# zju3dv/PVO

Hardware: AMD Instinct MI355X
Metric: VO keyframe updates/sec (8-keyframe window, 512x384, 36 edges; 6 graph updates + edge rebuild per keyframe) (higher is better)
Workload: dtype f16 (volume, lookup, update operator) / f32 (BA assembly) / f64 (pose solve); 1 GPU; S-B: BASELINE.json configs[1] window (8 keyframes, 48x64 maps, E=36, itrs=2), synthetic; edges=36, parallelism=independent window per GPU

## Files before the change

### include/pvo_hip.h

```cpp
#ifndef PVO_HIP_H
#define PVO_HIP_H

#include <stddef.h>
#include <stdint.h>

#ifdef __cplusplus
extern "C" {
#endif

enum { PVO_F32 = 0, PVO_F16 = 1, PVO_BF16 = 2, PVO_F64 = 3 };

enum {
  PVO_OK = 0,
  PVO_EINVAL = 1,
  PVO_ELAUNCH = 2,
  PVO_EWORKSPACE = 3,
  PVO_EUNSUPPORTED = 4
};

const char* pvo_strerror(int code);
const char* pvo_last_hip_error(void);
#define PVO_ABI_VERSION 106
int pvo_version(void);
size_t pvo_graph_update_args_size(void);
// ... 536 lines not shown
                 int t0, int t1, int iterations, float lm, float ep, int motion_only,
                 float* dx_out, float* dz_out, int dz_rows, int* status_out,
                 void* workspace, size_t workspace_bytes,
                 const float* disps_sens, float alpha, void* stream);
int pvo_ba_stereo(void* workspace, size_t workspace_bytes, int E, int P, int nframes, int HW, float baseline, void* stream);
int pvo_ba_rig(float* poses, float* disps, const float* intrinsics,
               const float* targets, const float* weights, const float* eta,
               const int64_t* ii, const int64_t* jj,
               int E, int nframes, int ht, int wd, int K_eta,
               int t0, int t1, int iterations, float lm, float ep, int motion_only,
               float* dx_out, float* dz_out, int dz_rows, int* status_out,
               void* workspace, size_t workspace_bytes,
               const float* disps_sens, float alpha, float baseline, void* stream);
int pvo_ba_last_partition(void* workspace, size_t workspace_bytes, int E, int P, int nframes, int HW, int* out, void* stream);
int pvo_ba_local(const float* poses, const float* disps, const float* intrinsics,
                 const float* targets, const float* weights, const float* eta,
                 const int64_t* ii, const int64_t* jj,
                 int E, int nframes, int ht, int wd, int K_eta, int t0, int t1,
                 int motion_only, void* sys,
                 void* workspace, size_t workspace_bytes, void* stream);
int pvo_ba_finish(float* poses, float* disps, void* sys,
                  const int64_t* ii, const int64_t* jj,
                  int E, int nframes, int ht, int wd, int t0, int t1,
                  float lm, float ep, int motion_only, int clamp_frames, float disp_min,
                  float* dx_out, float* dz_out, int dz_rows, int* status_out,
                  void* workspace, size_t workspace_bytes, void* stream);
int pvo_ba_finish_graph(float* poses, float* disps, void* sys,
                        const int64_t* ii, const int64_t* jj,
                        int E, int nframes, int ht, int wd, int t0, int t1,
                        float lm, float ep, int motion_only, int clamp_frames, float disp_min,
                        float* dx_out, float* dz_out, int dz_rows, int* status_out,
                        void* workspace, size_t workspace_bytes, int graph_edges, void* stream);
int pvo_ba_solve_kind(int P, int graph_edges, int packed);
int pvo_ba_sigma(const void* sys, void* workspace, size_t workspace_bytes,
                 const int64_t* ii, const int64_t* jj,
                 int E, int P, int nframes, int ht, int wd, int t0, float lm, float ep,
                 double* pose_cov, float* var_cond, float* var_pose, int* status_out, void* stream);
int pvo_ba_uncertainty(const float* poses, const float* disps, const float* intrinsics,
                       const float* targets, const float* weights, const float* eta,
                       const int64_t* ii, const int64_t* jj,
                       int E, int nframes, int ht, int wd, int K_eta,
                       int t0, int t1, float lm, float ep,
                       double* pose_cov, float* var_cond, float* var_pose, int* status_out,
                       void* workspace, size_t workspace_bytes,
                       const float* disps_sens, float alpha, float baseline, void* stream);
size_t pvo_ba_calib_workspace_bytes(int E, int P, int nframes, int HW);
int pvo_ba_calib(float* poses, float* disps, float* intrinsics,
                 const float* targets, const float* weights, const float* eta,
                 const int64_t* ii, const int64_t* jj,
                 int E, int nframes, int ht, int wd, int K_eta,
                 int t0, int t1, int iterations, float lm, float ep, float ep_c, int free_mask,
                 float* dx_out, float* dz_out, int dz_rows, float* dc_out, int* status_out,
                 void* workspace, size_t workspace_bytes, void* calib_workspace, size_t calib_bytes, void* stream);
size_t pvo_ba_packed_elems(const int* first_host, int P);
int pvo_ba_pack(void* sys, const int* first_s, void* msg, int P, void* stream);
int pvo_ba_finish_packed(float* poses, float* disps, const void* msg, const int* first_s,
                         const int64_t* ii, const int64_t* jj,
                         int E, int nframes, int ht, int wd, int t0, int t1,
                         float lm, float ep, int motion_only, int clamp_frames, float disp_min,
                         float* dx_out, float* dz_out, int dz_rows, int* status_out,
                         void* workspace, size_t workspace_bytes, void* stream);

typedef struct pvo_ba_riders {
  const void* cx; const void* cw; const float* cbias; void* cy; long long crows; int cCout; int cdtype;
  const void* gnet; const void* gw; const float* gbias; float* gpart; int gE; int gHW; int gdtype;
  const float* xpart; const float* xwt; const float* xbias; float* xg; int xE; int xchunks;
// ... 35 lines not shown
```

### pvo_amd/_lib.py

```python
import ctypes
import os

_HERE = os.path.dirname(os.path.abspath(__file__))
LIB_PATH = os.path.join(_HERE, "libpvo_hip.so")

PVO_F32, PVO_F16, PVO_BF16, PVO_F64 = 0, 1, 2, 3
PVO_ABI_VERSION = 106

_c = ctypes
_vp, _i, _f, _sz = _c.c_void_p, _c.c_int, _c.c_float, _c.c_size_t

SIGNATURES = {
    "pvo_strerror": (_c.c_char_p, [_i]),
    "pvo_version": (_i, []),
    "pvo_graph_update_args_size": (_sz, []),
    "pvo_last_hip_error": (_c.c_char_p, []),
    "pvo_debug_config": (_i, [_i, _i]),
    "pvo_knob": (_i, [_i]),
    "pvo_debug_trunk_range": (_i, [_i, _vp, _vp, _vp, _vp, _vp, _i, _i, _i, _i, _i, _i, _i, _i, _i, _vp, _i, _i, _vp]),
    "pvo_corr_index_forward": (_i, [_vp, _vp, _vp, _i, _i, _i, _i, _i, _i, _i, _vp]),
    "pvo_corr_index_backward": (_i, [_vp, _vp, _vp, _i, _i, _i, _i, _i, _i, _i, _vp]),
    "pvo_corr_pyramid_lookup": (_i, [_vp, _vp, _vp, _i, _i, _i, _i, _i, _i, _i, _i, _i, _vp, _i, _vp]),
    "pvo_altcorr_forward": (_i, [_vp, _vp, _vp, _vp, _i, _i, _i, _i, _i, _i, _i, _i, _i, _vp]),
    "pvo_altcorr_backward": (_i, [_vp, _vp, _vp, _vp, _vp, _vp, _i, _i, _i, _i, _i, _i, _i, _i, _i, _vp]),
# ... 96 lines not shown
    "pvo_tsdf_sparse_mesh_args_size": (_sz, []),
    "pvo_tsdf_sparse_mesh_workspace_bytes": (_sz, [_i]),
    "pvo_tsdf_sparse_mesh": (_i, [_vp, _vp, _sz, _vp]),
    "pvo_tsdf_panoptic_args_size": (_sz, []),
    "pvo_tsdf_mesh_labels_args_size": (_sz, []),
    "pvo_tsdf_integrate_panoptic": (_i, [_vp, _vp, _vp, _sz, _vp]),
    "pvo_tsdf_sparse_integrate_panoptic": (_i, [_vp, _vp, _vp, _sz, _vp]),
    "pvo_tsdf_mesh_panoptic": (_i, [_vp, _vp, _vp, _sz, _vp]),
    "pvo_tsdf_sparse_mesh_panoptic": (_i, [_vp, _vp, _vp, _sz, _vp]),
    "pvo_tsdf_render_args_size": (_sz, []),
    "pvo_tsdf_render_workspace_bytes": (_sz, [_i]),
    "pvo_tsdf_render": (_i, [_vp, _vp, _sz, _vp]),
    "pvo_tsdf_sparse_render_args_size": (_sz, []),
    "pvo_tsdf_sparse_render_workspace_bytes": (_sz, [_i]),
    "pvo_tsdf_sparse_render": (_i, [_vp, _vp, _sz, _vp]),
    "pvo_tsdf_track_args_size": (_sz, []),
    "pvo_tsdf_track_workspace_bytes": (_sz, [_i, _i, _i]),
    "pvo_tsdf_track": (_i, [_vp, _vp, _sz, _vp]),
    "pvo_tsdf_sparse_track_args_size": (_sz, []),
    "pvo_tsdf_sparse_track_workspace_bytes": (_sz, [_i, _i, _i]),
    "pvo_tsdf_sparse_track": (_i, [_vp, _vp, _sz, _vp]),
    "pvo_ba_last_partition": (_i, [_vp, _sz, _i, _i, _i, _i, ctypes.POINTER(ctypes.c_int), _vp]),
    "pvo_ba_packed_elems": (_sz, [ctypes.POINTER(ctypes.c_int), _i]),
    "pvo_ba_pack": (_i, [_vp, _vp, _vp, _i, _vp]),
    "pvo_ba_finish_packed": (_i, [_vp, _vp, _vp, _vp, _vp, _vp, _i, _i, _i, _i, _i, _i, _f, _f, _i, _i, _f,
                                  _vp, _vp, _i, _vp, _vp, _sz, _vp]),
    "pvo_ba_local": (_i, [_vp, _vp, _vp, _vp, _vp, _vp, _vp, _vp, _i, _i, _i, _i, _i, _i, _i,
                          _i, _vp, _vp, _sz, _vp]),
    "pvo_ba_finish": (_i, [_vp, _vp, _vp, _vp, _vp, _i, _i, _i, _i, _i, _i, _f, _f, _i, _i, _f,
                           _vp, _vp, _i, _vp, _vp, _sz, _vp]),
    "pvo_ba_finish_graph": (_i, [_vp, _vp, _vp, _vp, _vp, _i, _i, _i, _i, _i, _i, _f, _f, _i, _i, _f,
                                 _vp, _vp, _i, _vp, _vp, _sz, _i, _vp]),
    "pvo_ba_solve_kind": (_i, [_i, _i, _i]),
    "pvo_ba_finish_riders": (_i, [_vp, _vp, _vp, _vp, _vp, _i, _i, _i, _i, _i, _i, _f, _f, _i, _i, _f,
                                  _vp, _vp, _i, _vp, _vp, _sz, _vp, _vp]),
    "pvo_ba_finish_conv1x1": (_i, [_vp, _vp, _vp, _vp, _vp, _i, _i, _i, _i, _i, _i, _f, _f, _i, _i, _f,
                                   _vp, _vp, _i, _vp, _vp, _sz, _vp, _vp, _vp, _vp, _c.c_longlong, _i, _i, _vp]),
    "pvo_ba_train_workspace_bytes": (_sz, [_i, _i, _i, _i, _i, _i]),
    "pvo_ba_train_vjp_scratch_bytes": (_sz, [_i, _i, _i, _i, _i, _i]),
    "pvo_ba_train": (_i, [_vp, _vp, _vp, _vp, _vp, _vp, _vp, _vp, _vp, _vp, _vp, _vp, _i, _i, _i, _i, _i, _i, _i,
                          _vp, _vp, _vp, _vp, _sz, _i, _vp]),
    "pvo_ba_train_vjp": (_i, [_vp, _vp, _vp, _vp, _vp, _vp, _vp, _vp, _vp, _vp, _vp, _i, _i, _i, _i, _i, _i, _i,
                              _vp, _vp, _vp, _vp, _vp, _vp, _vp, _vp, _sz, _vp, _sz, _i, _vp]),
}



class UpdateWeights(_c.Structure):
    _fields_ = [("dtype", _i), ("flags", _i)] + [(n, _vp) for n in (
        "enc0_w", "enc0_b", "cenc2_w", "cenc2_b", "fenc0_w", "fenc0_b", "fenc2_w", "fenc2_b", "glo_w", "glo_b",
        "gate_wt", "gate_b", "zr_w", "q_w", "zr_inp_w", "q_inp_w", "heads1_w", "heads1_b", "heads2_w", "heads2_b",
        "agg1_w", "agg1_b", "agg2_w", "agg2_b", "eta_w", "eta_b", "up_w", "up_b")]


class OperatorArgs(_c.Structure):
    _fields_ = [("E", _i), ("H", _i), ("W", _i), ("levels", _vp * 4), ("slots", _vp), ("num_slots", _i),
                ("coords", _vp), ("corr", _vp), ("motion", _vp), ("net", _vp), ("net_out", _vp), ("inp", _vp),
                ("P_zr", _vp), ("P_q", _vp), ("static_by_slot", _i), ("seg_ptr", _vp), ("seg_idx", _vp), ("K", _i), ("heads", _vp),
                ("eta_frame", _vp), ("eta_pos", _vp), ("R", _i), ("damping", _vp), ("EP", _f), ("eta_scale", _f), ("eta", _vp),
                ("upmask", _vp)]


class GraphUpdateArgs(_c.Structure):
    _fields_ = [("op", OperatorArgs), ("nframes", _i), ("poses", _vp), ("disps", _vp), ("intrinsics", _vp),
                ("ii", _vp), ("jj", _vp), ("target", _vp), ("delta_dy", _vp), ("raw_mask", _vp), ("weight", _vp),
                ("full_flow", _vp), ("segm", _vp), ("max_segments", _i), ("vote_thresh", _f), ("dy_thresh", _f),
# ... 170 lines not shown
```

### pvo_amd/csrc/ba.hip

```cpp
#include "se3.h"
#include "conv1x1_tile.h"
#include "glo_tile.h"
#include <stdlib.h>
#include <type_traits>
#include "ba_workspace.h"
#include "ba_assemble.h"
#include "ba_schur.h"

namespace {

#ifdef PVO_BA_PROBE
__device__ unsigned long long* g_ba_probe = nullptr;
#define BA_PROBE(slot) do { if (g_ba_probe && threadIdx.x == 0) g_ba_probe[slot] = __builtin_readcyclecounter(); } while (0)
#else
#define BA_PROBE(slot)
#endif
#if defined(PVO_BA_PROBE) && PVO_BA_PROBE == 2
#define BA_PROBE_STEP(slot) do { if (g_ba_probe && lane == 0 && kb == P / 2) g_ba_probe[slot] = __builtin_readcyclecounter(); } while (0)
#else
#define BA_PROBE_STEP(slot)
#endif

__device__ __forceinline__ double rsqrt_nr(double d) {
  double y = __builtin_amdgcn_rsq(d);
// ... 1603 lines not shown
  __syncthreads();
  if (tid < 64) {
    for (int j = nc - 1; j >= 0; --j) {
      if (lane == j) xk[j] = s[j] * rinv[j];
      const double xj = xk[j];
      if (lane < j) s[lane] -= Lk[j][lane] * xj;
    }
  }
  __syncthreads();
  const int bj = blockIdx.x;
  if (bj == kb) {
    if (tid < nc) xvec[c0 + tid] = xk[tid];
    return;
  }
  if (tid < kNB) {
    const int col = kNB * bj + tid;
    double v = yrow[col];
    for (int r = 0; r < nc; ++r) v -= A[static_cast<size_t>(c0 + r) * n + col] * xk[r];
    yrow[col] = v;
  }
}

__global__ __launch_bounds__(256) void dense_finish_kernel(const double* __restrict__ xvec, float* __restrict__ poses, float* __restrict__ dx_ws,
                                                           float* __restrict__ dx_out, int* __restrict__ meta, int* __restrict__ status_out,
                                                           int P, int t0, Riders riders) {
  extern __shared__ __attribute__((aligned(16))) unsigned char smem[];
  if (blockIdx.x > 0) {
    ride(smem, riders, blockIdx.x - 1);
    return;
  }
  solve_epilogue([&](int i) { return xvec[i]; }, meta[4] | meta[2], true, 0, P, t0, poses, dx_ws, dx_out, meta, status_out, true, [] {});
}

template <bool CALIB>
__device__ __forceinline__ void ba_backsub_body(
    const Plan& pl, const int64_t* __restrict__ jj, const float* __restrict__ Ei, const float* __restrict__ Eij,
    const float* __restrict__ Q, const float* __restrict__ w, const float* __restrict__ dx,
    float* __restrict__ disps, float* __restrict__ dz_out, int dz_rows, int HW, int t0, int P,
    int clamp_frames, float disp_min, const float* __restrict__ Gc = nullptr, const float* __restrict__ dcw = nullptr) {
  const int k = blockIdx.y;
  const int x = blockIdx.x * 256 + threadIdx.x;
  __shared__ int s_edge[256], s_pose[256];
  __shared__ float s_dx[256][6];
  const bool live = k < pl.meta[0] && !pl.meta[2];
  const int e0 = live ? pl.eptr[k] : 0, deg = live ? pl.eptr[k + 1] - e0 : 0;
  const bool in_lds = deg <= 255;
  constexpr int lo = 1;
  if (live && in_lds && static_cast<int>(threadIdx.x) <= deg) {
    const int r = static_cast<int>(threadIdx.x) - 1;
    int e = 0, p;
    if (r < 0) p = pl.kx[k] - t0;
    else { e = pl.eidx[e0 + r]; p = static_cast<int>(jj[e]) - t0; }
    const bool ok = p >= 0 && p < P && p >= lo;
    s_edge[threadIdx.x] = e; s_pose[threadIdx.x] = ok ? p : -1;
#pragma unroll
    for (int n = 0; n < 6; ++n) s_dx[threadIdx.x][n] = ok ? dx[6 * p + n] : 0.0f;
  }
  BA_WG_PROBE(2, 0);
  __syncthreads();
  BA_WG_PROBE(2, 1);
  if (x >= HW) return;
  if (k < clamp_frames && pl.kidx[k] < 0) {
    const float v = disps[static_cast<long long>(k) * HW + x];
    if (v < disp_min) disps[static_cast<long long>(k) * HW + x] = disp_min;
  }
  if constexpr (CALIB) {
    if (k >= pl.meta[0]) return;
    if (!live || reinterpret_cast<const int*>(dcw)[4] != 0) {
      if (dz_out && k < dz_rows) dz_out[static_cast<long long>(k) * HW + x] = 0.0f;
      return;
    }
  }
  if (!live) return;
  float acc = 0.0f;
  if (in_lds) {
    for (int q = 0; q <= deg; ++q) {
      const int p = s_pose[q];
      if (p < 0) continue;
      const float* base = (q == 0) ? Ei + static_cast<long long>(p) * 6 * HW : Eij + static_cast<long long>(s_edge[q]) * 6 * HW;
      float sacc = 0.0f;
#pragma unroll
      for (int n = 0; n < 6; ++n) sacc += base[static_cast<long long>(n) * HW + x] * s_dx[q][n];
      acc += sacc;
    }
  } else {
    for (int r = -1; r < deg; ++r) {
      const RowRef R = row_of(r, k, pl, Ei, Eij, jj, HW, t0, P);
      if (R.pose < lo) continue;
      float sacc = 0.0f;
#pragma unroll
      for (int n = 0; n < 6; ++n) sacc += R.base[static_cast<long long>(n) * HW + x] * dx[6 * R.pose + n];
      acc += sacc;
    }
  }
  if constexpr (CALIB) {
    float cacc = 0.0f;
#pragma unroll
    for (int n = 0; n < 4; ++n) cacc += Gc[(static_cast<long long>(k) * 4 + n) * HW + x] * dcw[n];
    acc += cacc;
  }
  const float dz = Q[static_cast<long long>(k) * HW + x] * (w[static_cast<long long>(k) * HW + x] - acc);
  float d = disps[static_cast<long long>(pl.kx[k]) * HW + x] + dz;
  if (pl.kx[k] < clamp_frames && d < disp_min) d = disp_min;
  disps[static_cast<long long>(pl.kx[k]) * HW + x] = d;
  if (dz_out && k < dz_rows) dz_out[static_cast<long long>(k) * HW + x] = dz;
  BA_WG_PROBE(2, 2);
}

__global__ __launch_bounds__(256) void ba_backsub_kernel(
    Plan pl, const int64_t* __restrict__ jj, const float* __restrict__ Ei, const float* __restrict__ Eij,
    const float* __restrict__ Q, const float* __restrict__ w, const float* __restrict__ dx,
    float* __restrict__ disps, float* __restrict__ dz_out, int dz_rows, int HW, int t0, int P,
    int clamp_frames, float disp_min) {
  ba_backsub_body<false>(pl, jj, Ei, Eij, Q, w, dx, disps, dz_out, dz_rows, HW, t0, P, clamp_frames, disp_min);
}

constexpr int kSigmaMaxPoses = 64;
constexpr int kSigmaBlocks = 210;

__global__ __launch_bounds__(256) void ba_sigma_prepare_kernel(const long long* __restrict__ sys, double* __restrict__ out, int n, float lm, float ep) {
  const int idx = blockIdx.x * 256 + threadIdx.x;
  if (idx >= n * n) return;
  const int r = idx / n, c = idx - r * n;
  if (r > c) { out[idx] = 0.0; return; }
  double v = static_cast<double>(sys[static_cast<long long>(c) * n + r]) * kInvFix;
  if (r == c) v += static_cast<double>(ep) + static_cast<double>(lm) * v;
  out[idx] = v;
}

__global__ __launch_bounds__(1024) void ba_sigma_factor_kernel(double* R, int n, const int* __restrict__ meta, int* __restrict__ status_out) {
  __shared__ double s_col[8][8];
  int* flag = reinterpret_cast<int*>(R + static_cast<long long>(n) * n);
  double* rdiag = R + static_cast<long long>(n) * n + 1;
  const int tid = threadIdx.x, c = tid >> 7, il = tid & 127;
  int failed = (meta[2] | meta[3] | meta[4]) ? 1 : 0;
  for (int j0 = 0; j0 < n && !failed; j0 += 8) {
    const int j = j0 + c;
    double acc[3] = {0.0, 0.0, 0.0};
    for (int k0 = 0; k0 < j0; k0 += 8) {
      __syncthreads();
      if (tid < 64) s_col[tid >> 3][tid & 7] = (j0 + (tid & 7) < n) ? R[static_cast<long long>(k0 + (tid >> 3)) * n + j0 + (tid & 7)] : 0.0;
      __syncthreads();
#pragma unroll
      for (int kk = 0; kk < 8; ++kk) {
        const double a = s_col[kk][c];
        const double* row = R + static_cast<long long>(k0 + kk) * n;
#pragma unroll
        for (int u = 0; u < 3; ++u) {
// ... 675 lines not shown
    const bool stage2 = dense_window;
#define PVO_SCHUR_LAUNCH(V, PX) hipLaunchKernelGGL((ba_schur_mfma_kernel<V, PX>), sgrid, dim3(256), (PX == 256 ? sdyn : 0), st, w.plan, jj, eta, K_eta, w.Eii, w.Cii, w.bz, w.Ei, \
                                                   w.Eij, w.Q, w.w, sys, HW, t0, P, two_stage ? w.part : nullptr, ii, E, chunksA, deal_rows, w.Mrg, depth_done, (PX == 256 ? lds_floats : 0), \
                                                   (stage2 && PX == 256) ? w.spart : nullptr, w.srow, stage2 ? w.sT : nullptr, disps)
    if ((HW & 3) == 0) { if (pix == 256) PVO_SCHUR_LAUNCH(true, 256); else if (pix == 512) PVO_SCHUR_LAUNCH(true, 512); else PVO_SCHUR_LAUNCH(true, 1024); }
    else { if (pix == 256) PVO_SCHUR_LAUNCH(false, 256); else if (pix == 512) PVO_SCHUR_LAUNCH(false, 512); else PVO_SCHUR_LAUNCH(false, 1024); }
#undef PVO_SCHUR_LAUNCH
    PVO_CHECK_LAUNCH();
    if (stage2) {
      hipLaunchKernelGGL(ba_schur_reduce_kernel, dim3(kSchurStagePairs, Kgrid), dim3(256), 0, st, w.plan, w.spart, w.srow, w.sT, sys, gx, 6 * P, t0);
      PVO_CHECK_LAUNCH();
    }
  }
  return PVO_OK;
}

enum SolveKind { kSolveStatus, kSolveDense, kSolveEnvelope, kSolveChain, kSolveBlocks };
struct SolveForm { SolveKind kind; int chol; };
static SolveForm solve_form(int P, int E, bool packed, int knob) {
  if (P == 0) return {kSolveStatus, 0};
  if (knob >= 1 && knob <= 3) return {kSolveChain, knob - 1};
  if (knob == 4) return {kSolveEnvelope, 2};
  if (knob == 6 && !packed) return {kSolveBlocks, 0};
  if (P <= kDenseMaxPoses) return {kSolveDense, 0};
  if (knob != 5 && !packed && static_cast<long long>(E) > 8LL * P) return {kSolveBlocks, 0};
  return {kSolveEnvelope, 2};
}

extern "C" int pvo_ba_solve_kind(int P, int graph_edges, int packed) {
  if (P < 0 || graph_edges < 0) return -1;
  return static_cast<int>(solve_form(P, graph_edges, packed != 0, pvo_knob(PVO_KNOB_BA_SOLVER)).kind);
}

static int ba_finish_impl(float* poses, float* disps, void* sys_, const long long* msg, const int* first_s,
                          const int64_t* ii, const int64_t* jj,
                          int E, int nframes, int ht, int wd, int t0, int t1,
                          float lm, float ep, int motion_only, int clamp_frames, float disp_min,
                          float* dx_out, float* dz_out, int dz_rows, int* status_out,
                          void* workspace, size_t workspace_bytes,
                          const pvo_ba_riders* jobs, int graph_edges, void* stream) {
  Riders rider{};
  size_t rider_lds = 0;
  if (jobs && jobs->cy && jobs->crows > 0) {
    if (!jobs->cx || !jobs->cw || jobs->cCout <= 0 || jobs->cCout % 192) return PVO_EINVAL;
    if (jobs->cdtype != PVO_F16 && jobs->cdtype != PVO_BF16) return PVO_EUNSUPPORTED;
    if (pvo_misaligned16(jobs->cx, jobs->cw, jobs->cy)) return PVO_EINVAL;
    if (jobs->crows > (1LL << 24)) return PVO_EUNSUPPORTED;
    rider.cx = static_cast<const uint16_t*>(jobs->cx); rider.cw = static_cast<const uint16_t*>(jobs->cw); rider.cbias = jobs->cbias;
    rider.cy = static_cast<uint16_t*>(jobs->cy); rider.crows = jobs->crows; rider.cCout = jobs->cCout; rider.cdtype = jobs->cdtype;
    rider.crow_blocks = static_cast<int>((jobs->crows + 63) / 64);
    rider.cblocks = rider.crow_blocks * (jobs->cCout / 192);
    rider_lds = c1t::kTileBytes;
  }
  if (jobs && jobs->gpart && jobs->gE > 0 && jobs->gHW > 0) {
    if (!jobs->gnet || !jobs->gw || jobs->gE > 65535) return PVO_EINVAL;
    if (jobs->gdtype != PVO_F16 && jobs->gdtype != PVO_BF16) return PVO_EUNSUPPORTED;
    if (pvo_misaligned16(jobs->gnet, jobs->gw)) return PVO_EINVAL;
    rider.gnet = static_cast<const uint16_t*>(jobs->gnet); rider.gw = static_cast<const uint16_t*>(jobs->gw); rider.gbias = jobs->gbias;
    rider.gpart = jobs->gpart; rider.gHW = jobs->gHW; rider.gchunks = (jobs->gHW + 255) / 256; rider.gdtype = jobs->gdtype;
    rider.gblocks = jobs->gE * rider.gchunks;
    if (rider_lds < static_cast<size_t>(glt::kTileBytes)) rider_lds = glt::kTileBytes;
  }
  if (jobs && jobs->xg && jobs->xE > 0) {
    if (!jobs->xpart || !jobs->xwt || !jobs->xbias || jobs->xchunks <= 0) return PVO_EINVAL;
    rider.xpart = jobs->xpart; rider.xwt = jobs->xwt; rider.xbias = jobs->xbias; rider.xg = jobs->xg;
    rider.xchunks = jobs->xchunks; rider.xblocks = jobs->xE;
    if (rider_lds < 512) rider_lds = 512;
  }
  const int rider_blocks = rider.cblocks + rider.gblocks + rider.xblocks;
  int rc = check_common(E, nframes, ht, wd, t0, t1);
  if (rc != PVO_OK) return rc;
  if (clamp_frames < 0 || clamp_frames > nframes) return PVO_EINVAL;
  const int P = t1 - t0, HW = ht * wd;
  long long* sys = static_cast<long long*>(sys_);
  if (!poses || !disps || (!sys && !msg) || !workspace) return PVO_EINVAL;
  if (P > kMaxEnvBlocks) return PVO_EUNSUPPORTED;
  Ws w;
  if (!carve_checked(&w, workspace, workspace_bytes, E, P, nframes, HW)) return PVO_EWORKSPACE;
  hipStream_t st = pvo_stream(stream);
  const int n6 = 6 * P;
  const SolveForm form = solve_form(P, graph_edges >= 0 ? graph_edges : E, msg != nullptr, pvo_knob(PVO_KNOB_BA_SOLVER));
  if (msg && form.kind == kSolveStatus) return PVO_OK;
  constexpr size_t kSolveLdsMax = 142000;
  if (form.kind == kSolveDense) {
    const size_t dl = dense_lds_bytes(n6);
    const size_t lds = dl > rider_lds ? dl : rider_lds;
    const int Td = dense_N(n6) / 16;
    if (!pvo_allow_lds<ba_solve_dense_kernel<4>>(kSolveLdsMax) || !pvo_allow_lds<ba_solve_dense_kernel<14>>(kSolveLdsMax) ||
        !pvo_allow_lds<ba_solve_dense_kernel<17>>(kSolveLdsMax))
      return PVO_ELAUNCH;
    const auto kernel = Td <= 5 ? ba_solve_dense_kernel<4> : (Td <= 10 ? ba_solve_dense_kernel<14> : ba_solve_dense_kernel<17>);
    hipLaunchKernelGGL(kernel, dim3(1 + rider_blocks), dim3(256), lds, st, sys, msg, first_s, poses, w.dx, dx_out, w.plan.meta, status_out,
                       P, t0, lm, ep, rider);
  } else if (form.kind == kSolveEnvelope || form.kind == kSolveChain) {
    int* part = form.kind == kSolveEnvelope ? reinterpret_cast<int*>(w.xchg) : nullptr;
    if (msg) {
      hipLaunchKernelGGL(ba_env_packed_kernel, dim3(P), dim3(256), 0, st, msg, first_s, w.plan.env, n6);
      hipLaunchKernelGGL(ba_prepare_packed_kernel, dim3(P + 1), dim3(256), 0, st, msg, first_s, w.chol, w.plan.env, n6, lm, ep,
                         static_cast<long long>(kSolveLdsMax), part);
    } else {
      hipLaunchKernelGGL(ba_env_kernel, dim3((n6 * n6 + 2047) / 2048), dim3(256), 0, st, sys, w.plan.env, n6);
      hipLaunchKernelGGL(ba_prepare_kernel, dim3((n6 * n6 + n6 + 2047) / 2048), dim3(256), 0, st, sys, w.chol, w.plan.env, n6, lm, ep,
                         static_cast<long long>(kSolveLdsMax), part);
    }
    PVO_CHECK_LAUNCH();
    if (!part && hipMemsetAsync(w.xchg, 0, 16, st) != hipSuccess) return PVO_ELAUNCH;
    if (!pvo_allow_lds<ba_solve_twin_kernel>(kSolveLdsMax)) return PVO_ELAUNCH;
    hipLaunchKernelGGL(ba_solve_twin_kernel, dim3(2 + rider_blocks), dim3(256), kSolveLdsMax > rider_lds ? kSolveLdsMax : rider_lds, st,
                       w.chol, poses, w.dx, dx_out, w.plan.meta, status_out, P, t0, w.plan.env, static_cast<long long>(kSolveLdsMax), w.xchg,
                       form.chol, rider);
  } else {
    if (form.kind == kSolveBlocks) {
      hipLaunchKernelGGL(ba_prepare_kernel, dim3((n6 * n6 + n6 + 2047) / 2048), dim3(256), 0, st, sys, w.chol, w.plan.env, n6, lm, ep,
                         0LL , static_cast<int*>(nullptr));
      PVO_CHECK_LAUNCH();
      if (hipMemsetAsync(w.xchg, 0, 16, st) != hipSuccess) return PVO_ELAUNCH;
// ... 281 lines not shown
```

### pvo_amd/csrc/ba_workspace.h

```cpp
#pragma once
#include "common.h"

namespace {

constexpr float kMinDepth = 0.25f;

constexpr double kFix = 268435456.0, kInvFix = 1.0 / 268435456.0;
__device__ __forceinline__ void fix_add(long long* sys, long long idx, double v, int* meta) {
  if (!(fabs(v) < 3.0e10)) { meta[4] = 1; return; }
#ifdef PVO_BA_NO_ATOMICS
  if (idx >= 0) return;
#endif
  atomicAdd(reinterpret_cast<unsigned long long*>(sys + idx), static_cast<unsigned long long>(__double2ll_rn(v * kFix)));
}
constexpr int kDealEdges = 2;
constexpr int kPPT = 2;
constexpr int kChunkA = 256 * kPPT;
constexpr int kMaxSep = 12;
constexpr int kXchgDoubles = 2 + 36 * kMaxSep * kMaxSep + 12 * kMaxSep;


#if defined(PVO_BA_PROBE) && PVO_BA_PROBE == 3
__device__ unsigned long long* g_ba_wg_probe = nullptr;
#define BA_WG_PROBE(kern, slot)                                                                                         \
  do {                                                                                                                  \
    if (g_ba_wg_probe && threadIdx.x == 0 && blockIdx.z == 0) {                                                         \
      const unsigned wg_ = blockIdx.y * gridDim.x + blockIdx.x;                                                         \
      if (wg_ < 4096u) g_ba_wg_probe[((kern) * 4096u + wg_) * 8u + (slot)] = wall_clock64();                            \
    }                                                                                                                   \
  } while (0)
#else
#define BA_WG_PROBE(kern, slot)
#endif

struct Plan {
  int* kidx;
  int* kx;
  int* eptr;
  int* eidx;
  int* meta;
  int* env;
};

struct Ws {
  Plan plan;
  float *Eii, *Eij;
  float *Cii, *bz;
  float *Ei;
  float *Q, *w;
  float *dx;
  float *part;
  long long* sys;
  double* chol;
  double* xchg;
  double* ldiag;
  double* xvec;
  float* Mrg;
  float* spart;
  short* srow;
  int* sT;
  size_t bytes;
};
constexpr int kSchurStagePairs = 36;
constexpr int kSchurStageFront = 8;
__host__ __device__ __forceinline__ int schur_stage_frames(int P) { return (P > 0 && P <= 29) ? P + kSchurStageFront : 0; }
__host__ __device__ __forceinline__ int schur_stage_slot(int frame, int t0, int P) {
  const int slot = frame - t0 + kSchurStageFront;
  return (slot >= 0 && slot < schur_stage_frames(P)) ? slot : -1;
}

__host__ size_t align_up(size_t x) { return (x + 255) & ~static_cast<size_t>(255); }

__host__ Ws carve(void* base, int E, int P, int F, int HW) {
  Ws w{};
  char* p = static_cast<char*>(base);
// ... 69 lines not shown
  int cnt = 0;
  for (int f = lo; f < hi; ++f) cnt += pl.kidx[f];
  seg[tid + 1] = cnt;
  if (tid == 0) seg[0] = 0;
  __syncthreads();
  if (tid == 0) for (int i = 1; i <= 256; ++i) seg[i] += seg[i - 1];
  __syncthreads();
  int run = seg[tid];
  for (int f = lo; f < hi; ++f) {
    if (pl.kidx[f]) { pl.kx[run] = f; pl.kidx[f] = run; ++run; } else pl.kidx[f] = -1;
  }
  const int K = seg[256];
  __syncthreads();
  for (int k = tid; k < K; k += 256) {
    const int f = pl.kx[k];
    int c = 0;
    for (int e = 0; e < E; ++e) c += (ii[e] == f) ? 1 : 0;
    pl.eptr[k + 1] = c;
  }
  if (tid == 0) pl.eptr[0] = 0;
  __syncthreads();
  if (tid == 0) for (int k = 1; k <= K; ++k) pl.eptr[k] += pl.eptr[k - 1];
  __syncthreads();
  for (int k = tid; k < K; k += 256) {
    const int f = pl.kx[k];
    int o = pl.eptr[k];
    for (int e = 0; e < E; ++e) if (ii[e] == f) pl.eidx[o++] = e;
  }
  if (tid == 0) {
    pl.meta[0] = K;
    pl.meta[1] = 0;
    pl.meta[3] = 0;
    pl.meta[4] = 0;
    pl.meta[2] = (!motion_only && K_eta != K && K_eta != 1) ? 1 : 0;
    store_prior(pl.meta, sens, alpha);
    pl.meta[8] = __float_as_int(baseline);
  }
}

}
```

### pvo_amd/droid_backends.py

```python
import ctypes
import itertools

import torch

from . import _lib
from ._lib import PvoHipError, check

_DT = {torch.float32: _lib.PVO_F32, torch.float16: _lib.PVO_F16,
       torch.bfloat16: _lib.PVO_BF16, torch.float64: _lib.PVO_F64}

_ws_cache = {}


def _contig(t, name):
    if not t.is_contiguous():
        raise RuntimeError("%s must be contiguous" % name)


def _dev(*ts):
    dev = None
    for t in ts:
        if t is None:
            continue
        if not t.is_cuda:
# ... 1218 lines not shown
    if eta is not None:
        eta = eta.contiguous().view(-1, ht * wd)
        K_eta = eta.shape[0]
    with torch.cuda.device(dev):
        check(_lib.load().pvo_ba_local(_ptr(poses), _ptr(disps), _ptr(intrinsics), _ptr(targets), _ptr(weights),
                                       _ptr(eta) if eta is not None else ctypes.c_void_p(0), _ptr(ii), _ptr(jj),
                                       ii.shape[0], F, ht, wd, K_eta, int(t0), int(t1), (1 if motion_only else 0) | (2 if sys_is_zero else 0),
                                       _ptr(sys), ctypes.c_void_p(workspace.data_ptr()), workspace.numel(),
                                       _stream(dev)), "ba_local")


def ba_packed_elems(first):
    arr = (ctypes.c_int * len(first))(*[int(f) for f in first])
    return int(_lib.load().pvo_ba_packed_elems(arr, len(first)))


def ba_pack(sys, first_dev, msg):
    dev = _dev(sys, first_dev, msg)
    if sys.dtype != torch.int64 or msg.dtype != torch.int64 or first_dev.dtype != torch.int32:
        raise PvoHipError("ba_pack: sys / msg must be int64, first int32")
    with torch.cuda.device(dev):
        check(_lib.load().pvo_ba_pack(_ptr(sys), _ptr(first_dev), _ptr(msg), int(first_dev.shape[0]), _stream(dev)), "ba_pack")
    return msg


BA_SOLVE_KINDS = ("status", "dense", "envelope", "chain", "blocks")


def ba_solve_kind(P, graph_edges, packed=False):
    k = int(_lib.load().pvo_ba_solve_kind(int(P), int(graph_edges), 1 if packed else 0))
    if k < 0:
        raise PvoHipError("ba_solve_kind: P and graph_edges must not be negative")
    return BA_SOLVE_KINDS[k]


def ba_finish(poses, disps, sys, ii, jj, t0, t1, lm, ep, motion_only, workspace, dz_rows=0, status=None, outputs=True,
              clamp_frames=0, disp_min=0.001, rider=None, packed=None, graph_edges=None):
    dev = _dev(poses, disps, sys, ii, jj, workspace)
    rx = rw = rb = ry = None
    rrows = rC = rdt = 0
    if rider is not None:
        rx, rw, rb = rider
        _cl(rx, "rider x", 128)
        if rw.dim() != 2 or rw.shape[1] != 128 or rw.dtype != rx.dtype or not rw.is_contiguous():
            raise PvoHipError("ba_finish: rider w must be a contiguous [Cout,128] tensor in x's dtype")
        rC = rw.shape[0]
        ry = _new_cl(rx.shape[0], rC, rx.shape[2], rx.shape[3], rx.dtype, dev)
        rrows, rdt = rx.shape[0] * rx.shape[2] * rx.shape[3], _dtype_code(rx, "rider x")
    F, ht, wd = disps.shape
    P = int(t1) - int(t0)
    dx = torch.zeros(max(P, 0), 6, dtype=torch.float32, device=dev) if outputs else None
    dz = torch.zeros(int(dz_rows), ht * wd, dtype=torch.float32, device=dev) if outputs else None
    if not outputs:
        dz_rows = 0
    if packed is not None:
        msg, first_dev = packed
        if rider is not None:
            raise PvoHipError("ba_finish: a rider and a packed message together are not supported")
        if msg.dtype != torch.int64 or first_dev.dtype != torch.int32 or first_dev.shape[0] != P:
            raise PvoHipError("ba_finish: packed = (int64 message, int32 [P] structural envelope)")
        with torch.cuda.device(dev):
            check(_lib.load().pvo_ba_finish_packed(
                _ptr(poses), _ptr(disps), _ptr(msg), _ptr(first_dev), _ptr(ii), _ptr(jj), ii.shape[0], F, ht, wd,
                int(t0), int(t1), float(lm), float(ep), 1 if motion_only else 0,
                int(clamp_frames), float(disp_min), _ptr(dx), _ptr(dz), int(dz_rows),
                _ptr(status) if status is not None else ctypes.c_void_p(0),
# ... 977 lines not shown
```

Before: 265.6 keyframe updates/s.

## Fuse small dense pose solve with disparity back-substitution in one kernel

For small pose counts (P ≤ 10) with the default dense solver, the pose Cholesky solve and the per-pixel disparity back-substitution now run in a single kernel launch. Every block's first wave does a register-resident wave-level Cholesky on the reduced system, and the remaining waves prefetch that block's Ei/Eij/Q/w rows to warm the cache. A ticket counter picks the last block to clear the system and write the status. This removes a separate launch and serialization point, at the cost of redundant solve work in every block and extra atomics.

```diff
diff --git a/include/pvo_hip.h b/include/pvo_hip.h
--- a/include/pvo_hip.h
+++ b/include/pvo_hip.h
@@ -592,6 +592,7 @@
                         float* dx_out, float* dz_out, int dz_rows, int* status_out,
                         void* workspace, size_t workspace_bytes, int graph_edges, void* stream);
 int pvo_ba_solve_kind(int P, int graph_edges, int packed);
+int pvo_ba_finish_form(int P, int packed);
 int pvo_ba_sigma(const void* sys, void* workspace, size_t workspace_bytes,
                  const int64_t* ii, const int64_t* jj,
                  int E, int P, int nframes, int ht, int wd, int t0, float lm, float ep,
diff --git a/pvo_amd/_lib.py b/pvo_amd/_lib.py
--- a/pvo_amd/_lib.py
+++ b/pvo_amd/_lib.py
@@ -152,6 +152,7 @@
     "pvo_ba_finish_graph": (_i, [_vp, _vp, _vp, _vp, _vp, _i, _i, _i, _i, _i, _i, _f, _f, _i, _i, _f,
                                  _vp, _vp, _i, _vp, _vp, _sz, _i, _vp]),
     "pvo_ba_solve_kind": (_i, [_i, _i, _i]),
+    "pvo_ba_finish_form": (_i, [_i, _i]),
     "pvo_ba_finish_riders": (_i, [_vp, _vp, _vp, _vp, _vp, _i, _i, _i, _i, _i, _i, _f, _f, _i, _i, _f,
                                   _vp, _vp, _i, _vp, _vp, _sz, _vp, _vp]),
     "pvo_ba_finish_conv1x1": (_i, [_vp, _vp, _vp, _vp, _vp, _i, _i, _i, _i, _i, _i, _f, _f, _i, _i, _f,
diff --git a/pvo_amd/csrc/ba.hip b/pvo_amd/csrc/ba.hip
--- a/pvo_amd/csrc/ba.hip
+++ b/pvo_amd/csrc/ba.hip
@@ -1659,33 +1659,59 @@
   solve_epilogue([&](int i) { return xvec[i]; }, meta[4] | meta[2], true, 0, P, t0, poses, dx_ws, dx_out, meta, status_out, true, [] {});
 }
 
-template <bool CALIB>
+struct BacksubNoSolve { __device__ __forceinline__ const float* operator()(bool, int, int) const { return nullptr; } };
+template <bool CALIB, bool FUSED = false, class Solve = BacksubNoSolve>
 __device__ __forceinline__ void ba_backsub_body(
     const Plan& pl, const int64_t* __restrict__ jj, const float* __restrict__ Ei, const float* __restrict__ Eij,
     const float* __restrict__ Q, const float* __restrict__ w, const float* __restrict__ dx,
     float* __restrict__ disps, float* __restrict__ dz_out, int dz_rows, int HW, int t0, int P,
-    int clamp_frames, float disp_min, const float* __restrict__ Gc = nullptr, const float* __restrict__ dcw = nullptr) {
-  const int k = blockIdx.y;
-  const int x = blockIdx.x * 256 + threadIdx.x;
+    int clamp_frames, float disp_min, const float* __restrict__ Gc = nullptr, const float* __restrict__ dcw = nullptr,
+    int fused_bx = 0, int fused_k = 0, bool fused_backsub = true, Solve solve = Solve{}) {
+  const int k = FUSED ? fused_k : static_cast<int>(blockIdx.y);
+  const int x = (FUSED ? fused_bx : static_cast<int>(blockIdx.x)) * 256 + threadIdx.x;
   __shared__ int s_edge[256], s_pose[256];
   __shared__ float s_dx[256][6];
-  const bool live = k < pl.meta[0] && !pl.meta[2];
-  const int e0 = live ? pl.eptr[k] : 0, deg = live ? pl.eptr[k + 1] - e0 : 0;
-  const bool in_lds = deg <= 255;
+  bool live = false, in_lds = true;
+  int e0 = 0, deg = 0;
+  auto head = [&]() __attribute__((always_inline)) {
+    live = (!FUSED || fused_backsub) && k < pl.meta[0] && !pl.meta[2];
+    e0 = live ? pl.eptr[k] : 0; deg = live ? pl.eptr[k + 1] - e0 : 0;
+    in_lds = deg <= 255;
+  };
+  const bool solver_wave = FUSED && __builtin_amdgcn_readfirstlane(static_cast<int>(threadIdx.x) >> 6) == 0;
+  if (!solver_wave) head();
   constexpr int lo = 1;
-  if (live && in_lds && static_cast<int>(threadIdx.x) <= deg) {
-    const int r = static_cast<int>(threadIdx.x) - 1;
+  auto table_row = [&](int q, bool with_dx) {
+    const int r = q - 1;
     int e = 0, p;
     if (r < 0) p = pl.kx[k] - t0;
     else { e = pl.eidx[e0 + r]; p = static_cast<int>(jj[e]) - t0; }
     const bool ok = p >= 0 && p < P && p >= lo;
-    s_edge[threadIdx.x] = e; s_pose[threadIdx.x] = ok ? p : -1;
-#pragma unroll
-    for (int n = 0; n < 6; ++n) s_dx[threadIdx.x][n] = ok ? dx[6 * p + n] : 0.0f;
-  }
-  BA_WG_PROBE(2, 0);
+    s_edge[q] = e; s_pose[q] = ok ? p : -1;
+    if (with_dx) {
+#pragma unroll
+      for (int n = 0; n < 6; ++n) s_dx[q][n] = ok ? dx[6 * p + n] : 0.0f;
+    }
+  };
+  if constexpr (!FUSED) {
+    if (live && in_lds && static_cast<int>(threadIdx.x) <= deg) table_row(threadIdx.x, true);
+    BA_WG_PROBE(2, 0);
+  } else {
+    if (live && in_lds) for (int q = static_cast<int>(threadIdx.x) - 64; q <= deg; q += 192) if (q >= 0) table_row(q, false);
+    BA_WG_PROBE(2, 0);
+    dx = solve(live, e0, deg);
+    if (solver_wave) head();
+    if (live && in_lds) {
+      for (int q = threadIdx.x; q <= deg; q += 256) {
+        const int p = s_pose[q];
+#pragma unroll
+        for (int n = 0; n < 6; ++n) s_dx[q][n] = p >= 0 ? dx[6 * p + n] : 0.0f;
+      }
+    }
+  }
   __syncthreads();
   BA_WG_PROBE(2, 1);
+  if (FUSED && !fused_backsub) return;
   if (x >= HW) return;
   if (k < clamp_frames && pl.kidx[k] < 0) {
     const float v = disps[static_cast<long long>(k) * HW + x];
@@ -1741,6 +1767,194 @@
     int clamp_frames, float disp_min) {
   ba_backsub_body<false>(pl, jj, Ei, Eij, Q, w, dx, disps, dz_out, dz_rows, HW, t0, P, clamp_frames, disp_min);
 }
+
+constexpr int kSmallMaxPoses = 10;
+
+__device__ __forceinline__ double lane_bcast(double v, int l) {
+  const long long b = __double_as_longlong(v);
+  const int lo = __builtin_amdgcn_readlane(static_cast<int>(b & 0xffffffffLL), l);
+  const int hi = __builtin_amdgcn_readlane(static_cast<int>(b >> 32), l);
+  return __longlong_as_double((static_cast<long long>(hi) << 32) | static_cast<unsigned int>(lo));
+}
+
+struct SmallRow { const long long *row, *rhs; int cmin, cmax; };
+__device__ __forceinline__ SmallRow small_row(const long long* sys, const long long* msg, const int* first_s, int P, int row) {
+  const int n = 6 * P;
+  SmallRow r;
+  r.cmax = row < n ? row : (row == n ? n - 1 : -1);
+  r.cmin = 0;
+  if (!msg) { r.row = sys + (row <= n ? row * n : 0); r.rhs = sys; return r; }
+  const int rb = row < n ? row / 6 : P;
+  int run = 0, total = 0, f = 0;
+  for (int b = 0; b < P; ++b) {
+    const int e = first_s[b];
+    const int fb = e < b ? (e < 0 ? 0 : e) : b;
+    if (b < rb) run += (b - fb + 1) * 36;
+    total += (b - fb + 1) * 36;
+    if (b == rb) f = fb;
+  }
+  r.row = row < n ? msg + (run - 36 * f + 6 * (row - 6 * rb)) : msg;
+  r.rhs = msg + total;
+  if (row < n) r.cmin = 6 * f;
+  return r;
+}
+
+template <int N, bool MSG>
+__device__ __forceinline__ void small_load(const SmallRow& R, int lane, float lm, float ep, double (&a)[6 * kSmallMaxPoses]) {
+  constexpr int B = N < 30 ? N : 30;
+  const long long* __restrict__ rhs = R.rhs;
+#pragma unroll
+  for (int c0 = 0; c0 < N; c0 += B) {
+    long long raw[B];
+#pragma unroll
+    for (int u = 0; u < B; ++u) {
+      const int c = c0 + u < N ? c0 + u : N - 1;
+      long long v = R.row[c + (MSG ? 30 : 0) * (c / 6)];
+      if (MSG) { const long long y = rhs[c]; v = lane == N ? y : v; }
+      raw[u] = (c >= R.cmin && c <= R.cmax) ? v : 0LL;
+    }
+#pragma unroll
+    for (int u = 0; u < B; ++u) {
+      const int c = c0 + u;
+      if (c >= N) continue;
+      double v = static_cast<double>(raw[u]) * kInvFix;
+      if (c == lane) v += static_cast<double>(ep) + static_cast<double>(lm) * v;
+      a[c] = v;
+    }
+  }
+}
+
+template <int J, int N>
+__device__ __forceinline__ void chol_small_column(double (&a)[6 * kSmallMaxPoses], int lane, bool& ok, double& myrs) {
+  if constexpr (J < N) {
+    const double d = lane_bcast(a[J], J);
+    ok = ok && d > 0.0;
+    const double rs = ok ? rsqrt_nr1(d) : 0.0;
+    myrs = lane == J ? rs : myrs;
+    const double l = a[J] * rs;
+    a[J] = l;
+#pragma unroll
+    for (int k = J + 1; k < N; ++k) a[k] = __builtin_fma(-l, lane_bcast(l, k), a[k]);
+    chol_small_column<J + 1, N>(a, lane, ok, myrs);
+  }
+}
+
+template <int PP, class Loaded>
+__device__ __forceinline__ double chol_solve_small(const SmallRow& R, bool packed, int lane, float lm, float ep, Loaded loaded, double* __restrict__ Ls, int* failed) {
+  constexpr int n = 6 * PP, pitch = n | 1;
+  double a[6 * kSmallMaxPoses];
+  if (packed) small_load<n, true>(R, lane, lm, ep, a); else small_load<n, false>(R, lane, lm, ep, a);
+  loaded();
+  bool ok = true;
+  double myrs = 0.0;
+  chol_small_column<0, n>(a, lane, ok, myrs);
+  *failed = ok ? 0 : 1;
+  if (lane <= n) {
+#pragma unroll
+    for (int c = 0; c < n; ++c) Ls[lane * pitch + c] = a[c];
+  }
+  __builtin_amdgcn_fence(__ATOMIC_RELEASE, "wavefront");
+  __builtin_amdgcn_wave_barrier();
+  __builtin_amdgcn_fence(__ATOMIC_ACQUIRE, "wavefront");
+  const int col = lane < n ? lane : 0;
+  double z = lane < n ? Ls[n * pitch + col] : 0.0;
+#pragma unroll 6
+  for (int j = n - 1; j >= 0; --j) {
+    const double l = Ls[j * pitch + col];
+    const double xj = lane_bcast(z * myrs, j);
+    z = lane < j ? __builtin_fma(-l, xj, z) : (lane == j ? xj : z);
+  }
+  return z;
+}
+
+struct SmallFinish {
+  long long* sys; const long long* msg; const int* first_s;
+  float *poses, *dx_ws, *dx_out; int* status_out;
+  int P, t0; float lm, ep;
+  Plan pl; const int64_t* jj; const float *Ei, *Eij, *Q, *w; float *disps, *dz_out;
+  int dz_rows, HW, clamp_frames; float disp_min;
+  int gx, nba, backsub;
+};
+
+#define PVO_SMALL_SIZES(X) X(1) X(2) X(3) X(4) X(5) X(6) X(7) X(8) X(9) X(10)
+__device__ __forceinline__ void small_finish(const SmallFinish& A, unsigned char* smem, int b) {
+  const int PP = A.P, n = 6 * PP;
+  __shared__ float s_dxv[64];
+  __shared__ int s_fail, s_last;
+  int* meta = A.pl.meta;
+  const int tid = threadIdx.x, lane = tid & 63, wave = __builtin_amdgcn_readfirstlane(tid >> 6);
+  const int bx = b % A.gx, k = b / A.gx;
+  auto solve = [&](bool live, int e0, int deg) __attribute__((always_inline)) -> const float* {
+    if (wave == 0) {
+      const int bad = meta[4] | meta[2];
+      const SmallRow R = small_row(A.sys, A.msg, A.first_s, PP, lane);
+      auto loaded = [&]() __attribute__((always_inline)) {
+        __threadfence();
+        if (lane == 0) s_last = atomicAdd(&meta[kMetaTicket], 1) == A.nba - 1 ? 1 : 0;
+      };
+      int fail = 0;
+      double x = 0.0;
+      double* Ls = reinterpret_cast<double*>(smem);
+      switch (PP) {
+#define PVO_SMALL_SOLVE(K) case K: x = chol_solve_small<K>(R, A.msg != nullptr, lane, A.lm, A.ep, loaded, Ls, &fail); break;
+        PVO_SMALL_SIZES(PVO_SMALL_SOLVE)
+#undef PVO_SMALL_SOLVE
+        default: loaded(); fail = 1; break;
+      }
+      const int failed = fail | bad;
+      float v = 0.0f;
+      if (!failed) v = !(x == x) ? 0.0f : static_cast<float>(x);
+      s_dxv[lane] = lane < n ? v : 0.0f;
+      if (lane == 0) s_fail = failed;
+    } else if (live) {
+      const int u = tid - 64, px0 = bx * 256;
+      float sink = 0.0f;
+      for (int L = u; L < (deg + 1) * 48; L += 192) {
+        const int q = L / 48, r = L - 48 * q, px = px0 + 32 * (r & 7);
+        if (px >= A.HW) continue;
+        int e = 0, p;
+        if (q == 0) p = A.pl.kx[k] - A.t0;
+        else { e = A.pl.eidx[e0 + q - 1]; p = static_cast<int>(A.jj[e]) - A.t0; }
+        if (p < 1 || p >= PP) continue;
+        const float* base = q == 0 ? A.Ei + static_cast<long long>(p) * 6 * A.HW : A.Eij + static_cast<long long>(e) * 6 * A.HW;
+        sink += base[static_cast<long long>(r >> 3) * A.HW + px];
+      }
+      if (u < 24 && px0 + 32 * (u & 7) < A.HW) {
+        const int px = px0 + 32 * (u & 7);
+        const float* arr = u < 8 ? A.Q + static_cast<long long>(k) * A.HW
+                                 : (u < 16 ? A.w + static_cast<long long>(k) * A.HW : A.disps + static_cast<long long>(A.pl.kx[k]) * A.HW);
+        sink += arr[px];
+      }
+      asm volatile("" ::"v"(sink));
+    }
+    __syncthreads();
+    return s_dxv;
+  };
+  ba_backsub_body<false, true>(A.pl, A.jj, A.Ei, A.Eij, A.Q, A.w, nullptr, A.disps, A.dz_out, A.dz_rows, A.HW, A.t0, PP,
+                               A.clamp_frames, A.disp_min, nullptr, nullptr, bx, k, A.backsub != 0, solve);
+  const int failed = s_fail;
+  if (b == 0)
+    solve_epilogue([&](int i) { return static_cast<double>(s_dxv[i]); }, failed, true, 0, PP, A.t0, A.poses, A.dx_ws, A.dx_out, meta,
+                   A.status_out, false, [] {});
+  if (s_last) {
+    __threadfence();
+    if (!A.msg) for (int idx = tid; idx < n * n + n; idx += 256) A.sys[idx] = 0LL;
+    if (tid == 0) {
+      meta[4] = 0;
+      if (failed) meta[1] = 1;
+      if (A.status_out) { A.status_out[0] = meta[1]; A.status_out[1] = meta[0]; A.status_out[2] = meta[2]; A.status_out[3] = meta[3]; }
+      meta[kMetaTicket] = 0;
+    }
+  }
+}
+
+__global__ __launch_bounds__(256) __attribute__((amdgpu_waves_per_eu(2))) void ba_solve_backsub_kernel(SmallFinish A, Riders riders) {
+  extern __shared__ __attribute__((aligned(16))) unsigned char smem[];
+  const int b = blockIdx.x;
+  if (b >= A.nba) { ride(smem, riders, b - A.nba); return; }
+  small_finish(A, smem, b);
+}
+__host__ __forceinline__ size_t small_lds_bytes(int P) { const size_t n = 6 * static_cast<size_t>(P); return sizeof(double) * (n + 1) * (n | 1); }
 
 constexpr int kSigmaMaxPoses = 64;
 constexpr int kSigmaBlocks = 210;
@@ -2482,6 +2696,14 @@
   return static_cast<int>(solve_form(P, graph_edges, packed != 0, pvo_knob(PVO_KNOB_BA_SOLVER)).kind);
 }
 
+static bool finish_fused(int P, bool packed, int knob) {
+  return knob == 0 && P >= 1 && P <= kSmallMaxPoses && solve_form(P, 0, packed, knob).kind == kSolveDense;
+}
+extern "C" int pvo_ba_finish_form(int P, int packed) {
+  if (P < 0) return -1;
+  return finish_fused(P, packed != 0, pvo_knob(PVO_KNOB_BA_SOLVER)) ? 1 : 0;
+}
+
 static int ba_finish_impl(float* poses, float* disps, void* sys_, const long long* msg, const int* first_s,
                           const int64_t* ii, const int64_t* jj,
                           int E, int nframes, int ht, int wd, int t0, int t1,
@@ -2532,6 +2754,26 @@
   const SolveForm form = solve_form(P, graph_edges >= 0 ? graph_edges : E, msg != nullptr, pvo_knob(PVO_KNOB_BA_SOLVER));
   if (msg && form.kind == kSolveStatus) return PVO_OK;
   constexpr size_t kSolveLdsMax = 142000;
+  if (form.kind == kSolveDense && finish_fused(P, msg != nullptr, pvo_knob(PVO_KNOB_BA_SOLVER))) {
+    SmallFinish A{};
+    A.sys = sys; A.msg = msg; A.first_s = first_s; A.poses = poses; A.dx_ws = w.dx; A.dx_out = dx_out; A.status_out = status_out;
+    A.P = P; A.t0 = t0; A.lm = lm; A.ep = ep;
+    A.pl = w.plan; A.jj = jj; A.Ei = w.Ei; A.Eij = w.Eij; A.Q = w.Q; A.w = w.w; A.disps = disps; A.dz_out = dz_out;
+    A.dz_rows = dz_rows; A.HW = HW; A.clamp_frames = clamp_frames; A.disp_min = disp_min;
+    A.backsub = (!motion_only && E + P > 0) ? 1 : 0;
+    const int Kmax = (nframes < P + E) ? nframes : (P + E);
+    A.gx = (HW + 255) / 256;
+    const long long rows = Kmax > clamp_frames ? Kmax : clamp_frames;
+    const long long nba = A.backsub ? A.gx * rows : 1;
+    if (nba + rider_blocks > 0x7fffffffLL) return PVO_EUNSUPPORTED;
+    A.nba = static_cast<int>(nba);
+    const size_t sl = small_lds_bytes(P);
+    const size_t lds = sl > rider_lds ? sl : rider_lds;
+    if (lds > 48 * 1024 && !pvo_allow_lds<ba_solve_backsub_kernel>(kSolveLdsMax)) return PVO_ELAUNCH;
+    hipLaunchKernelGGL(ba_solve_backsub_kernel, dim3(static_cast<unsigned>(nba + rider_blocks)), dim3(256), lds, st, A, rider);
+    PVO_CHECK_LAUNCH();
+    return PVO_OK;
+  }
   if (form.kind == kSolveDense) {
     const size_t dl = dense_lds_bytes(n6);
     const size_t lds = dl > rider_lds ? dl : rider_lds;
diff --git a/pvo_amd/csrc/ba_workspace.h b/pvo_amd/csrc/ba_workspace.h
--- a/pvo_amd/csrc/ba_workspace.h
+++ b/pvo_amd/csrc/ba_workspace.h
@@ -41,6 +41,8 @@
   int* meta;
   int* env;
 };
+
+constexpr int kMetaTicket = 9;
 
 struct Ws {
   Plan plan;
@@ -176,6 +178,7 @@
     pl.meta[1] = 0;
     pl.meta[3] = 0;
     pl.meta[4] = 0;
+    pl.meta[kMetaTicket] = 0;
     pl.meta[2] = (!motion_only && K_eta != K && K_eta != 1) ? 1 : 0;
     store_prior(pl.meta, sens, alpha);
     pl.meta[8] = __float_as_int(baseline);
diff --git a/pvo_amd/droid_backends.py b/pvo_amd/droid_backends.py
--- a/pvo_amd/droid_backends.py
+++ b/pvo_amd/droid_backends.py
@@ -1274,6 +1274,16 @@
     if k < 0:
         raise PvoHipError("ba_solve_kind: P and graph_edges must not be negative")
     return BA_SOLVE_KINDS[k]
+
+
+BA_FINISH_FORMS = ("separate", "fused")
+
+
+def ba_finish_form(P, packed=False):
+    k = int(_lib.load().pvo_ba_finish_form(int(P), 1 if packed else 0))
+    if k < 0:
+        raise PvoHipError("ba_finish_form: P must not be negative")
+    return BA_FINISH_FORMS[k]
 
 
 def ba_finish(poses, disps, sys, ii, jj, t0, t1, lm, ep, motion_only, workspace, dz_rows=0, status=None, outputs=True,
```

Measured after the change: 261.7 keyframe updates/s. -1.5%, worse.
